# sholtodouglas/RoboticsPlayroomPybullet

Measured on AMD Instinct MI355X. Metric: env-steps/sec at N=4096 parallel UR5PlayAbsRPY1Obj-v0 envs per MI355X, higher is better.
Workload: dtype f32

## Files before the change

roboticsplayroompybullet_amd/csrc/rp_kernels.cuh:

```cuda
#pragma once
#include <hip/hip_runtime.h>
#include <stdint.h>

#include "rp_device_model.h"
#include "rp_math.cuh"

#define NB_MAX (1 + RP_MAX_ARM + RP_MAX_FREE + RP_MAX_J1)
#define NVP 28
#define MAXC 21
#define MAXACT 64
#define MAXT 4
#define MAXROWC (3 * MAXC + MAXT)
static_assert(MAXACT <= 64 && NB_MAX <= 32, "a candidate record packs its pair index in 6 bits and its bodies in 5 bits each");
#define PM_MAX 11
#define PMC_HDR 4
#define PMC_PT 11
#define PMC_MAN (8 + 4 * PMC_PT)
#define PMC_MANIFOLDS (PMC_HDR + PM_MAX * PMC_MAN)
#define PMC_AX PMC_MANIFOLDS
#define PMC_AXN 16
#define PMC_FLOATS (PMC_MANIFOLDS + 8 * PMC_AXN)
#define RP_MAX_GROUPS 16
#define SORT_KEYS 64
#define SORT_REPS 8
// ... 3 lines not shown
#define RP_MAX_ENVS (1 << SORT_RANK_BITS)
#define MAXSMALL 44

#ifndef RP_PREP_WAVES
#define RP_PREP_WAVES 4
#endif
#ifndef RP_WAVES_PER_EU
#define RP_WAVES_PER_EU 1
#endif

#define K_DT (1.0f / 300.0f)
#define K_GRAVITY (-9.8f)
#define K_NSUB 12
#define K_NSETTLE 100
#define K_MAXVEL 100.0f
#ifdef K_NITER_OVERRIDE
#define K_NITER K_NITER_OVERRIDE
#else
#define K_NITER 50
#endif
#define K_ERP 0.08f
#define K_SLOP 1e-5f
#define K_TIE_EPS 1e-6f
#define K_KP 0.1f
#define K_DEFMOTOR 1.0f
#define K_LIMIT_MAXIMP 100.0f
#define K_ERP_LIMIT 0.2f
#define K_LIMIT_ACTIVATION 0.1f
#define K_LIN_DAMP 0.04f
#define K_ANG_DAMP 0.04f
#define K_IK_DAMP 0.1f
#define K_IK_RES 1e-4f
#define K_IK_MAXSTEP (45.0f * RP_PI_F / 180.0f)

#define ROWW 18
#define ROWREG ((ROWW * MAXROWC + 3) & ~3)

#ifdef RP_WIDE
#define O_FLOATS 160
#else
#define O_FLOATS 128
#endif
#define CANDMAX 64
#define MANPTS (MAXC + 3)
#define NPSCR_FLOATS 768
#define PREP_CH 8

#define HULL_POOL_FIELDS int hinfo[MAXACT][4]; int hout[MAXACT]; float hpt[MAXACT][7]; unsigned long long hcls[PMC_AXN];
struct __align__(16) EnvLds {
  float st[RP_REC_FLOATS];
  float xR[NB_MAX * 9], xp[NB_MAX * 3];
  float O[4];
  float S[RP_MAX_ARM * 6];
  float Minv[144], tau[RP_MAX_ARM];
  float finv[RP_MAX_FREE * 9];
  float dmu[RP_MAX_OBJ], dmass[RP_MAX_FREE + 1];
  float vstar[32];
  float conp[MAXC * 3], conn[MAXC * 3], cond[MAXC], conmu[MAXC];
  int cona[MAXC], conb[MAXC], conk[MAXC];
  int torc[MAXT]; float tors[MAXT];
  alignas(16) float srow[MAXSMALL * 8];
  alignas(16) float rowS[MAXROWC * 4];
  alignas(16) float rowT[MAXROWC * 4];
  union alignas(16) {
    struct {
      float aabb[RP_MAX_COL * 8];
      int act[MAXACT], candn[MAXACT], key[MAXACT];
      float pmu[MAXACT];
      alignas(16) float cand[CANDMAX * 8];
      alignas(16) float man[MANPTS * 8];
      float npscr[NPSCR_FLOATS];
      HULL_POOL_FIELDS
    };
    struct {
      float inert[RP_MAX_ARM * 10], compI[RP_MAX_ARM * 10];
      float vsp[RP_MAX_ARM * 6], csp[RP_MAX_ARM * 6], fsp[RP_MAX_ARM * 6], Fv[RP_MAX_ARM * 6];
      double Md[144];
    };
    struct { float J[ROWREG]; float B[ROWREG]; };
  };
  alignas(16) float out[O_FLOATS];
};

struct __align__(16) PrepLds {
  float st[RP_REC_FLOATS];
  int roff[64];
  int slot[64];
  unsigned amask[4];
  int hdr[4];
  float O[4];
  float S[RP_MAX_ARM * 6];
  float xR[NB_MAX * 9], xp[NB_MAX * 3];
  float conp[MAXC * 3], conn[MAXC * 3], cond[MAXC], conmu[MAXC];
  int cona[MAXC], conb[MAXC], conk[MAXC];
  int torc[MAXT]; float tors[MAXT];
  union alignas(16) {
    float aabb[RP_MAX_COL * 8];
    float npscr[NPSCR_FLOATS];
    float man[MANPTS * 8];
  };
  int act[MAXACT], candn[MAXACT], key[MAXACT];
  float pmu[MAXACT];
  alignas(16) float cand[CANDMAX * 8];
  alignas(16) float Minv[144];
  float tau[RP_MAX_ARM];
  float finv[RP_MAX_FREE * 9];
  float dmu[RP_MAX_OBJ], dmass[RP_MAX_FREE + 1];
  float vstar[32];
  union alignas(16) {
    struct {
      float inert[RP_MAX_ARM * 10], compI[RP_MAX_ARM * 10];
      float vsp[RP_MAX_ARM * 6], csp[RP_MAX_ARM * 6], fsp[RP_MAX_ARM * 6], Fv[RP_MAX_ARM * 6];
      double Md[144];
    };
    struct {
      float srow[MAXSMALL * 8];
      float rowS[3 * PREP_CH * 4], rowT[3 * PREP_CH * 4];
      union {
        struct { float J[3 * PREP_CH * ROWW], B[3 * PREP_CH * ROWW]; };
        float aout[192];
      };
    };
  };
  HULL_POOL_FIELDS
#ifdef RP_LDS_PAD
  float pad[RP_LDS_PAD];
#endif
};
static_assert(offsetof(EnvLds, aabb) % 16 == 0 && offsetof(PrepLds, aabb) % 16 == 0 && offsetof(EnvLds, cand) % 16 == 0 && offsetof(EnvLds, man) % 16 == 0 && offsetof(EnvLds, srow) % 16 == 0 && offsetof(EnvLds, rowS) % 16 == 0 &&
              offsetof(EnvLds, rowT) % 16 == 0 && offsetof(EnvLds, J) % 16 == 0 && offsetof(EnvLds, B) % 16 == 0, "16-byte LDS accesses");
static_assert(sizeof(PrepLds) <= 20480 - 512, "k_prep2: eight blocks (sixteen waves: what its 128 VGPRs allow) per CU");
static_assert(offsetof(PrepLds, roff) % 16 == 0 && offsetof(PrepLds, slot) % 16 == 0 && offsetof(PrepLds, Minv) % 16 == 0 && offsetof(PrepLds, aout) % 16 == 0 &&
              offsetof(PrepLds, Md) % 8 == 0 && offsetof(PrepLds, cand) % 16 == 0 && offsetof(PrepLds, man) % 16 == 0, "16-byte copies out of LDS");

struct __align__(16) ObsLds {
  float st[RP_REC_FLOATS];
  float xR[NB_MAX * 9], xp[NB_MAX * 3];
  float O[4];
  float S[RP_MAX_ARM * 6];
  alignas(16) float cand[2 * 12 * RP_MAX_ARM + 2 * RP_MAX_ARM + 4];
  alignas(16) float out[O_FLOATS];
};
#ifdef RP_CLOCKS
__device__ unsigned long long g_clk[32 * 4096];
#define CLK_MARK(i) if (lane == 0) { g_clk[8 * wb + (i)] = __builtin_readcyclecounter(); }
#if RP_CLOCKS == 2
#define PCLK(i) if (lane == 0) { g_clk[32 * (blockIdx.x & 4095) + (i)] = (i) >= 6 && (i) < 8 ? wall_clock64() : __builtin_readcyclecounter(); }
#define PCLK_ZERO(i) if (lane == 0) { g_clk[32 * (blockIdx.x & 4095) + (i)] = 0ull; }
#define PCLK_ADD(i, v) if (lane == 0) { g_clk[32 * (blockIdx.x & 4095) + (i)] += (unsigned long long)(v); }
#define HCLK_ADD(i, v) if (l16 == 0) { atomicAdd(&g_clk[32 * (blockIdx.x & 4095) + (i)], (unsigned long long)(v)); }
#ifdef RP_HPROF
#define PCLK_G(i, v)
#define PCLK_H(i, v) PCLK_ADD(i, v)
#else
#define PCLK_G(i, v) PCLK_ADD(i, v)
#define PCLK_H(i, v)
#endif
#define CLK_MARK2(i)
#else
#define PCLK(i)
#define PCLK_ZERO(i)
#define PCLK_ADD(i, v)
#define HCLK_ADD(i, v)
#define PCLK_G(i, v)
#define PCLK_H(i, v)
#define CLK_MARK2(i) CLK_MARK(i)
#endif
#else
#define CLK_MARK(i)
#define CLK_MARK2(i)
#define PCLK(i)
#define PCLK_ZERO(i)
#define PCLK_ADD(i, v)
#define HCLK_ADD(i, v)
#define PCLK_G(i, v)
#define PCLK_H(i, v)
#endif

#define WSYNC() do { __builtin_amdgcn_fence(__ATOMIC_RELEASE, "workgroup"); __builtin_amdgcn_wave_barrier(); __builtin_amdgcn_fence(__ATOMIC_ACQUIRE, "workgroup"); } while (0)

__device__ __forceinline__ int dof_free(const DevModel* m, int k) { return m->n_arm + 6 * k; }
__device__ __forceinline__ int dof_j1(const DevModel* m, int k) { return m->n_arm + 6 * m->n_free + k; }
#ifndef RP_WIDE
#define LANE_J1 16
#define LANE_FREE 19
__device__ __forceinline__ int lane_pos(const DevModel* m, int d) {
  if (d < m->n_arm) return d;
  const int e = d - m->n_arm, f6 = 6 * m->n_free;
  if (e >= f6) return LANE_J1 + (e - f6);
  const int f = e / 6, c = e - 6 * f;
  if ((m->free_row0 >> f) & 1) return c < 3 ? m->n_arm + c : -1;
  return LANE_FREE + e;
}
__device__ __forceinline__ int lane_dof(const DevModel* m, int l) {
  if (l < 16) {
    if (l < m->n_arm) return l;
    const int c = l - m->n_arm;
    return (m->free_row0 != 0 && c < 3) ? m->n_arm + 6 * (__ffs(m->free_row0) - 1) + c : -1;
  }
  if (l >= 32) return -1;
  if (l < LANE_FREE) return l - LANE_J1 < m->n_j1 ? m->n_arm + 6 * m->n_free + (l - LANE_J1) : -1;
  const int e = l - LANE_FREE, f = e / 6;
  return (e < 6 * m->n_free && !((m->free_row0 >> f) & 1)) ? m->n_arm + e : -1;
}
#else
#define LANE_J1 16
#define LANE_FREE 19
__device__ __forceinline__ int lane_pos(const DevModel* m, int d) {
  if (d < m->n_arm) return d;
  const int e = d - m->n_arm, f6 = 6 * m->n_free;
  if (e >= f6) return LANE_J1 + (e - f6);
  const int f = e / 6, c = e - 6 * f;
  return f == m->drawer_free ? m->n_arm + c : LANE_FREE + 6 * f + c;
}
// ... 1790 lines not shown
        V3 rxn = tors ? d : cross(rr, d);
        float im = 1.f / L.dmass[k];
        M3 Ii = ldm3(&L.finv[9 * k]);
        V3 w = mulv(Ii, rxn);
        const V3 dl = tors ? mk3(0, 0, 0) : d;
        float jl[3] = {sign * dl.x, sign * dl.y, sign * dl.z}, ja[3] = {sign * rxn.x, sign * rxn.y, sign * rxn.z};
        float ba[3] = {sign * w.x, sign * w.y, sign * w.z};
        for (int i = 0; i < 3; i++) {
          J[base + i] = jl[i]; B[base + i] = jl[i] * im; J[base + 3 + i] = ja[i]; B[base + 3 + i] = ba[i];
          diag += jl[i] * jl[i] * im + ja[i] * ba[i];
          relv += jl[i] * L.vstar[dd + i] + ja[i] * L.vstar[dd + 3 + i];
        }
        if (base == 0) off0 = dd; else off1 = dd;
      } else {
        int k = body - 1 - n - m->n_free, dd = dof_j1(m, k);
        M3 R = ldm3(&L.xR[9 * body]);
        V3 a = mulv(R, ld3(m->j1_axis[k]));
        float j = tors ? (m->j1_type[k] == 1 ? 0.f : sign * dot(a, d)) : (m->j1_type[k] == 1 ? sign * dot(d, a) : sign * dot(a, cross(p - ld3(m->j1_pos[k]), d)));
        float minv = m->j1_minv[k];
        J[base] = j; B[base] = j * minv;
        diag += j * j * minv; relv += j * L.vstar[dd];
        if (base == 0) off0 = dd; else off1 = dd;
      }
    }
    if (has_arm) {
      off0 = 0;
#pragma unroll
      for (int k = 0; k < RP_MAX_ARM; k++) if (k < n) J[k] = Jr[k];
    }
    float* s = &L.rowS[4 * r];
    s[0] = diag; s[1] = relv; s[2] = dir == 0 ? 0.f : (tors ? L.tors[r - nc] : L.conmu[ci]); s[3] = __int_as_float(dir == 0 ? 0 : ci);
    float* t = &L.rowT[4 * r];
    t[0] = __int_as_float(has_arm ? 1 : 0); t[1] = dir == 0 ? 1e10f : 0.f; t[2] = __int_as_float(off0); t[3] = __int_as_float(off1);
  }
  WSYNC();
  for (int e = lane; e < nrows * n; e += 64) {
    int r = e / n, i = e - r * n;
    if (__float_as_int(L.rowT[4 * r]) != 0) {
      const float* J = &L.J[r * ROWW];
      const float* Mi = &L.Minv[i * 12];
      float b = 0.f;
#pragma unroll
      for (int k = 0; k < RP_MAX_ARM; k++) { const float t = Mi[k] * J[k]; b = k < n ? b + t : b; }
      L.B[r * ROWW + i] = b;
    }
  }
  WSYNC();
  for (int r = lane; r < nrows; r += 64) {
    float* s = &L.rowS[4 * r];
    float* t = &L.rowT[4 * r];
    float diag = s[0], relv = s[1];
    if (__float_as_int(t[0]) != 0) {
      const float* J = &L.J[r * ROWW];
      const float* B = &L.B[r * ROWW];
#pragma unroll
      for (int i = 0; i < RP_MAX_ARM; i++) { const float jb = J[i] * B[i], jv = J[i] * L.vstar[i]; diag = i < n ? diag + jb : diag; relv = i < n ? relv + jv : relv; }
    }
    float dinv, rhs, cfmr = 0.f;
    if (r < nc) {
      const int ci = c0 + r;
      float cfm = 0.f, erp = K_ERP;
      float s0 = m->col_stiff[L.cona[ci]], s1 = m->col_stiff[L.conb[ci]];
      if (s0 > 0.f || s1 > 0.f) {
        float d0 = s0 > 0.f ? m->col_damp[L.cona[ci]] : 0.1f, d1 = s1 > 0.f ? m->col_damp[L.conb[ci]] : 0.1f;
        if (!(s0 > 0.f)) s0 = 1e18f;
        if (!(s1 > 0.f)) s1 = 1e18f;
        float ks = 1.f / (1.f / s0 + 1.f / s1), kd = d0 + d1;
        cfm = 1.f / (K_DT * (K_DT * ks + kd));
        erp = (K_DT * ks) / (K_DT * ks + kd);
      }
      dinv = safe_inv(diag + cfm);
      cfmr = cfm * dinv;
      float pen = L.cond[ci] + K_SLOP, pos_err = 0.f, vel_err = -relv;
      if (pen > 0.f) vel_err -= pen / K_DT; else pos_err = -pen * erp / K_DT;
      rhs = (pos_err + vel_err) * dinv;
    } else { dinv = safe_inv(diag); rhs = -relv * dinv; }
    s[0] = rhs; s[1] = cfmr;
    t[0] = __int_as_float((__float_as_int(t[0]) != 0 && __float_as_int(t[3]) != 64) ? 1 : 0);
    float* Jw = &L.J[r * ROWW];
    for (int k = 0; k < ROWW; k++) Jw[k] *= dinv;
  }
}

__device__ __forceinline__ float pgs_update(float delta, float lam, float lo, float hi, float& lam_out) {
  float d = __builtin_amdgcn_fmed3f(delta, lo - lam, hi - lam);
  lam_out = lam + d;
  return d;
}

template <class LDS>
__device__ float solve_rows(const DevModel* m, LDS& L, int lane, int nsmall_, int ncon_, int nt_) {
  const int n = m->n_arm;
  const int nsmall = uni(nsmall_), nrc = uni(3 * ncon_ + nt_);
  float dv = 0.f;
  float lamS = 0.f, lamC0 = 0.f, lamC1 = 0.f;
  for (int it = 0; it < K_NITER; it++) {
    {
      for (int rr = 0; rr < nsmall; rr++) {
        const int r = (it & 1) ? rr : nsmall - 1 - rr;
        const float4 c0 = *(const float4*)&L.srow[8 * r], c1 = *(const float4*)&L.srow[8 * r + 4];
        const int type_ = uni(__float_as_int(c0.x)), dA = uni(__float_as_int(c0.y)), dB = uni(__float_as_int(c1.w));
        const int type = type_ == SR_LIMIT ? SR_UNIT : type_;
        const float sg = c0.z, jA = c1.x;
        float bl = 0.f;
        if (type == SR_J1) bl = lane == lane_pos(m, dA) ? sg : 0.f;
        else if (lane < n) bl = type == SR_UNIT ? sg * L.Minv[lane * 12 + dA] : L.Minv[lane * 12 + dA] + sg * L.Minv[lane * 12 + dB];
        float delta;
        if (type == SR_UNIT) delta = __fmaf_rn(-(sg * jA), lane_read(dv, dA), c0.w);
        else if (type == SR_J1) delta = __fmaf_rn(-jA, lane_read(dv, uni(lane_pos(m, dA))), c0.w);
        else { float pa = jA * lane_read(dv, dA); float pb = (sg * jA) * lane_read(dv, dB); float jdv = pa + pb; delta = c0.w - jdv; }
        float lam = lane_read(lamS, r), lnew;
        const float d = pgs_update(delta, lam, c1.y, c1.z, lnew);
        lamS = lane == r ? lnew : lamS;
        dv = fmaf(bl, d, dv);
      }
    }
    if (nrc > 0) {
      float4 sn = *(const float4*)&L.rowS[0], tn = *(const float4*)&L.rowT[0];
      float4 s2 = sn, t2 = tn;
      if (nrc > 1) { s2 = *(const float4*)&L.rowS[4]; t2 = *(const float4*)&L.rowT[4]; }
      float jn = 0.f, bn = 0.f;
      const int mydof = lane_dof(m, lane);
      {
        int i1 = mydof - __float_as_int(tn.w), i0 = mydof - __float_as_int(tn.z);
        int idx = (unsigned)i1 < 6u ? 12 + i1 : ((unsigned)i0 < 12u ? i0 : -1);
        if (idx >= 0 && mydof >= 0) { jn = L.J[idx]; bn = L.B[idx]; }
      }
      for (int r = 0; r < nrc; r++) {
        float jl = jn, bl = bn;
        float rhs = sn.x, cfmr = sn.y, mu = sn.z, lo_c = 0.f, hi_c = tn.y;
        int parent = uni(__float_as_int(sn.w));
        sn = s2; tn = t2;
        if (r + 1 < nrc) {
          int i1 = mydof - __float_as_int(tn.w), i0 = mydof - __float_as_int(tn.z);
          int idx = (unsigned)i1 < 6u ? 12 + i1 : ((unsigned)i0 < 12u ? i0 : -1);
          jn = 0.f; bn = 0.f;
          if (idx >= 0 && mydof >= 0) { jn = L.J[(r + 1) * ROWW + idx]; bn = L.B[(r + 1) * ROWW + idx]; }
          if (r + 2 < nrc) { s2 = *(const float4*)&L.rowS[4 * (r + 2)]; t2 = *(const float4*)&L.rowT[4 * (r + 2)]; }
        }
        float lamv = r < 64 ? lamC0 : lamC1;
        float lam = lane_read(lamv, r & 63);
        const float tot = lane_read(lamC0, parent);
        float lim = mu * tot;
        float prod = jl * dv;
        float jdv = wave_sum32(prod), lnew;
        float d = pgs_update(__fmaf_rn(-lam, cfmr, rhs) - jdv, lam, lo_c - lim, hi_c + lim, lnew);
        if (r >= uni(ncon_) && !(tot > 0.f)) { d = 0.f; lnew = lam; }
        float sel = lane == (r & 63) ? lnew : lamv;
        lamC0 = r < 64 ? sel : lamC0;
        lamC1 = r < 64 ? lamC1 : sel;
        dv = fmaf(bl, d, dv);
      }
    }
  }
  return dv;
}

__device__ bool substep_heavy(const DevModel* m, EnvLds& L, int lane, int nsmall, int ncon, int nt);
__device__ void substep(const DevModel* m, EnvLds& L, int lane, int env) {
  int n = m->n_arm;
  stage_dynamics(m, L, lane, env);
  fk_bodies(m, L, lane);
  __syncthreads();
  joint_subspaces(m, L, lane);
  collider_aabbs(m, L, lane);
  __syncthreads();
// ... 889 lines not shown
    float aj = 0.f;
#pragma unroll
    for (int j = 0; j < 7; j++) aj = l16 == j ? a8[j] : aj;
    qj = at == RP_ACT_REL_JOINTS ? aj + q0 : aj;
  } else {
    V3 cp = mk3(0, 0, 0); Q4 cq = {0.f, 0.f, 0.f, 1.f};
    if (at == RP_ACT_REL_RPY || at == RP_ACT_REL_QUAT) ee_pose_coop(m, qj, l16, cp, cq);
    V3 tpos; Q4 tq;
    action_target(at, a8, cp, cq, tpos, tq);
    if (m->arm_type == RP_ARM_PANDA) qj = ik_coop<7>(m, tpos, tq, qj, 200, l16, live, &ik_capped, &ik_marginal);
    else if (nc == 6) { for (int rep = 0; rep < 4; rep++) qj = ik_coop<6>(m, tpos, tq, qj, 20, l16, live, &ik_capped, &ik_marginal); }
    else { for (int rep = 0; rep < 4; rep++) qj = ik_coop<7>(m, tpos, tq, qj, 20, l16, live, &ik_capped, &ik_marginal); }
  }
  if (!live) return;
  if (l16 < nd) {
    float t = clampf(qj, m->ll[l16], m->ul[l16]);
    t = clampf(t, q0 - m->inc[l16], q0 + m->inc[l16]);
    st[ST_MMODE + l16] = 1.f; st[ST_MTARGET + l16] = t; st[ST_MMAXIMP + l16] = 240.f * K_DT;
    if (target_poses) target_poses[(size_t)env * nd + l16] = t;
  }
  if (l16 == 0) {
    st[ST_STATUS] = __int_as_float((ik_capped ? 8 : 0) | (ik_marginal ? 16 : 0));
    float g = a8[m->n_action - 1];
    if (m->arm_type == RP_ARM_PANDA) {
      float amt = 0.04f - g / 25.f;
      int ds[2] = {m->d9p, m->d10p};
      for (int i = 0; i < 2; i++) { st[ST_MMODE + ds[i]] = 1.f; st[ST_MTARGET + ds[i]] = amt; st[ST_MMAXIMP + ds[i]] = 100.f * K_DT; }
    } else {
      float amt = g - 0.2f;
      float left = st[ST_Q + m->d18];
      int ds[6] = {m->d18, m->d20, m->d12, m->d15, m->d10, m->d13};
      float tg[6] = {amt * 0.055f, left, amt * 0.5f, amt * 0.5f, amt * 0.8f, amt * 0.8f};
      float fo[6] = {100.f, 1000.f, 100.f, 100.f, 100.f, 100.f};
      for (int i = 0; i < 6; i++) { st[ST_MMODE + ds[i]] = 1.f; st[ST_MTARGET + ds[i]] = tg[i]; st[ST_MMAXIMP + ds[i]] = fo[i] * K_DT; }
    }
  }
}

__global__ void __launch_bounds__(64) k_action(const DevModel* __restrict__ m, float* __restrict__ state, const float* __restrict__ action,
                                              float* __restrict__ target_poses, int env0, int N, const int* __restrict__ member) {
  action_body(m, state, action, target_poses, env0, N, member, blockIdx.x);
}

__device__ __forceinline__ void copy_out(float* __restrict__ dst, const float* src, int nfloat, int lane) {
  for (int i = lane * 4; i < nfloat; i += 256) *(float4*)(dst + i) = *(const float4*)(src + i);
}

#define NBJ 3
#define LBL_N NBJ
#define NLBL (LBL_N + MAXC)
#define GEAR_LANE 12
#define W3_HDR 0
#define W3_VSTAR 8
#define W3_MU 40
#define W3_MINV 72
#define W3_A 216
#define W3_GEAR (W3_A + 160)
#define W3_ZERO (W3_GEAR + 7)
#define W3_BJ (W3_GEAR + 8)
#define W3_ROWS (W3_BJ + 20)
#define W3_ROWT (W3_ROWS + 4 * MAXROWC)
#define W3_ROFF (W3_ROWT + 4 * MAXROWC)
#define W3_SLOT (W3_ROFF + 64)
#define W3_J (W3_SLOT + 64)
#define W3_B (W3_J + ROWREG)
#define W3_SROW (W3_B + ROWREG)
#define W3_FLOATS (W3_SROW + 4 + 8 * MAXSMALL)
#define STAGE_FLOATS (128 + 2 * ROWREG)
#define AOUT_FLOATS (160 + 8 + 20)
static_assert(W3_A % 4 == 0 && W3_ROWS % 4 == 0 && W3_ROFF % 4 == 0 && AOUT_FLOATS % 4 == 0, "16-byte copies");

#define HV_MAXC 14
#ifndef S4_SLOTS0
#define S4_SLOTS0 8
#endif
#ifndef S4_SLOTS1
#define S4_SLOTS1 8
#endif
__device__ __forceinline__ int hv_class(int nc, int nA, int nB, int nC) {
  const bool heavy = nC != 0 || nA > S4_SLOTS0 || nB > S4_SLOTS1;
  return !heavy ? 0 : (nc <= HV_MAXC ? 1 : 2);
}
#define PREP_THREADS 128
__device__ __forceinline__ void prep2_core(PrepLds& L, const DevModel* __restrict__ m, const float* __restrict__ state, float* __restrict__ ws, const int env, const int cenv,
                                           int* __restrict__ pair_tab, const int pair_idx, int* __restrict__ hv_cnt = nullptr, int* __restrict__ hv_list = nullptr, const int prep_flags = 0) {
  const int tid = threadIdx.x, wid = tid >> 6, lane = tid & 63;
  PCLK(6) PCLK(0) PCLK_ZERO(15) PCLK_ZERO(19) PCLK_ZERO(26) PCLK_ZERO(27) PCLK_ZERO(28) PCLK_ZERO(29) PCLK_ZERO(30) PCLK_ZERO(31)
  static_assert(RP_REC_FLOATS == PREP_THREADS, "one float of the record per thread");
  L.st[tid] = state[(size_t)env * RP_REC_FLOATS + tid];
  if (tid == 64) L.hdr[3] = pair_idx;
  if (tid == 64 && m->persist) L.hdr[2] = __float_as_int(m->pmcache[(size_t)cenv * PMC_FLOATS]);
  stage_dynamics(m, L, tid, cenv);
  __syncthreads();
  PCLK(16)
  if (wid == 0) fk_bodies(m, L, lane);
  __syncthreads();
  PCLK(17)
  float* w = ws + (size_t)env * W3_FLOATS;
  if (wid == 0) {
    collider_aabbs(m, L, lane);
    WSYNC();
    PCLK(1)
    int ncon = collide<PrepLds>(m, L, lane, cenv, &L.hdr[2]);
    ncon = uni(ncon);
#ifdef RP_ABL_MAXCON
    if (ncon > RP_ABL_MAXCON) ncon = RP_ABL_MAXCON;
#endif
    if (lane == 0) L.hdr[0] = ncon;
    PCLK(2)
  } else {
    joint_subspaces(m, L, lane);
    PCLK(18)
    arm_dynamics(m, L, lane, cenv);
    unconstrained_velocities(m, L, lane, cenv);
    PCLK(3)
    int nsmall = build_small_rows(m, L, lane);
    nsmall = uni(nsmall);
    for (int i = lane; i < AOUT_FLOATS; i += 64) L.aout[i] = 0.f;
    if (lane < 2) L.amask[lane] = 0u;
    if (lane == 2) L.amask[2] = (unsigned)nsmall;
    WSYNC();
    bool gear = false;
    if (lane < nsmall) {
      const float* s = &L.srow[8 * lane];
      int type = __float_as_int(s[0]), dA = __float_as_int(s[1]);
      float sg = s[2], rhs = s[3], dinv = s[4], lo = s[5], hi = s[6];
      if (type == SR_UNIT) {
        L.aout[dA] = dinv; L.aout[16 + dA] = rhs; L.aout[32 + dA] = lo; L.aout[48 + dA] = hi;
      } else if (type == SR_LIMIT) {
        int pl = sg > 0.f ? 64 : 112;
        L.aout[pl + dA] = sg * rhs; L.aout[pl + 16 + dA] = sg * lo; L.aout[pl + 32 + dA] = sg * hi;
        atomicOr(&L.amask[sg > 0.f ? 0 : 1], 1u << dA);
      } else if (type == SR_J1) {
        int k = lane;
        if (k < NBJ) { float* bq = &L.aout[168]; bq[k] = dinv; bq[4 + k] = rhs; bq[8 + k] = lo; bq[12 + k] = hi; bq[16 + k] = sg; }
      } else {
        float* g = &L.aout[160];
        g[0] = s[1]; g[1] = s[7]; g[2] = sg; g[3] = dinv; g[4] = rhs; g[5] = lo; g[6] = hi;
        gear = true;
      }
    }
    const bool anygear = __ballot(gear) != 0ull;
    if (lane == 0) L.hdr[1] = anygear ? 1 : 0;
    WSYNC();
    if (lane < 32) w[W3_VSTAR + lane] = L.vstar[lane];
    copy_out(w + W3_MINV, L.Minv, 144, lane);
    copy_out(w + W3_A, L.aout, AOUT_FLOATS, lane);
  }
  __syncthreads();
  const int ncon = L.hdr[0];
  int tid_j = threadIdx.x;
  asm volatile("" : "+v"(tid_j));
  const int wid_j = tid_j >> 6;
  if (wid_j == 0) {
    const int lane = tid_j & 63;
    float* w = ws + (size_t)env * W3_FLOATS;
    const int cls = lane < ncon ? L.conk[lane] : 3;
    const unsigned long long mB = __ballot(cls == 0), mA = __ballot(cls == 1), mC = __ballot(cls == 2);
    const unsigned long long lower = (1ull << lane) - 1ull;
    L.slot[lane] = -1;
    L.roff[lane] = 0;
    const int nt = tors_list(m, L, lane, ncon);
    WSYNC();
    if (cls == 0) L.slot[__popcll(mB & lower)] = lane;
    else if (cls == 1) L.slot[21 + __popcll(mA & lower)] = lane;
    else if (cls == 2) L.slot[42 + __popcll(mC & lower)] = lane;
    bool tors_done = nt == 0;
    for (int c0 = 0; c0 < ncon || !tors_done; c0 += PREP_CH) {
      const int nc = max(0, min(PREP_CH, ncon - c0));
      const int ntl = (!tors_done && c0 + PREP_CH >= ncon && 3 * nc + nt <= 3 * PREP_CH) ? nt : 0;
      contact_rows(m, L, lane, c0, nc, ntl);
      WSYNC();
      auto global_row = [&](int lr) { return lr < nc ? c0 + lr : (lr < nc + ntl ? 3 * ncon + (lr - nc) : ncon + 2 * c0 + (lr - nc - ntl)); };
      for (int e = lane; e < (3 * nc + ntl) * ROWW; e += 64) {
        const int lr = e / ROWW, k = e - lr * ROWW;
        const int gr = global_row(lr);
        w[W3_J + gr * ROWW + k] = L.J[e]; w[W3_B + gr * ROWW + k] = L.B[e];
      }
      for (int e = lane; e < (3 * nc + ntl) * 4; e += 64) {
        const int lr = e >> 2, k = e & 3;
        const int gr = global_row(lr);
        float v = L.rowS[e];
        if (k == 3 && lr >= nc && lr < nc + ntl) {
          const int c = L.torc[lr - nc], kc = L.conk[c];
          const unsigned long long mk = kc == 1 ? mA : (kc == 2 ? mC : mB);
          v = __int_as_float(c | (kc << 8) | (__popcll(mk & ((1ull << c) - 1ull)) << 12));
        }
        w[W3_ROWS + gr * 4 + k] = v; w[W3_ROWT + gr * 4 + k] = L.rowT[e];
      }
      if (lane < 3 * nc + ntl && !(lane >= nc && lane < nc + ntl)) {
        const int gr = global_row(lane);
        L.roff[gr] = __float_as_int(L.rowT[4 * lane + 2]) | (__float_as_int(L.rowT[4 * lane + 3]) << 8);
      }
      if (ntl > 0) tors_done = true;
      WSYNC();
    }
    PCLK(4)
    if (lane == 0) {
      int nj = m->n_j1 < NBJ ? m->n_j1 : NBJ;
      w[W3_HDR] = __int_as_float((int)L.amask[0]); w[W3_HDR + 1] = __int_as_float((int)L.amask[1]);
      w[W3_HDR + 2] = __int_as_float(nj); w[W3_HDR + 3] = __int_as_float(ncon);
      w[W3_HDR + 4] = __int_as_float(__popcll(mA)); w[W3_HDR + 5] = __int_as_float(__popcll(mB));
      w[W3_HDR + 6] = __int_as_float(L.hdr[1] | (nt << 8)); w[W3_HDR + 7] = __int_as_float(__popcll(mC));
      if (hv_list != nullptr && (hv_class(ncon, __popcll(mA), __popcll(mB), __popcll(mC)) != 0 || (prep_flags & 1))) hv_list[atomicAdd(hv_cnt, 1)] = env | (ncon << 24);
    }
    if (lane < 32) w[W3_MU + lane] = lane < ncon ? L.conmu[lane] : 0.f;
    copy_out(w + W3_ROFF, (const float*)L.roff, 64, lane);
    copy_out(w + W3_SLOT, (const float*)L.slot, 64, lane);
  } else {
    if ((tid_j & 63) == 0) pair_tab[L.hdr[3]] = env | (ncon << 24);
    if (prep_flags & 1) {
      const int lane = tid_j & 63;
      float* w = ws + (size_t)env * W3_FLOATS;
      const int nsm = (int)L.amask[2];
      if (lane == 0) w[W3_SROW] = __int_as_float(nsm);
      for (int i = lane; i < 8 * nsm; i += 64) w[W3_SROW + 4 + i] = L.srow[i];
    }
  }
  PCLK(5) PCLK(7)
}
__device__ __forceinline__ void prep2_body(const DevModel* __restrict__ m, const float* __restrict__ state, float* __restrict__ ws, int env0, int N,
                                           const int* __restrict__ sort_cnt, int* __restrict__ sort_cnt_next, const int* __restrict__ sort_slot, int* __restrict__ pair_env,
                                           const int* __restrict__ member, const int bid, const int* __restrict__ cache_env = nullptr, int* __restrict__ hv_cnt = nullptr, int* __restrict__ hv_cnt_next = nullptr,
                                           int* __restrict__ hv_list = nullptr, const int prep_flags = 0) {
  __shared__ PrepLds L;
  const int tid = threadIdx.x, wid = tid >> 6, lane = tid & 63;
  int env = env0 + bid;
  if (env >= N) return;
  if (member) env = member[env];
  if (bid == 0) {
    for (int i = tid; i < SORT_BINS; i += PREP_THREADS) sort_cnt_next[i] = 0;
    if (tid == 0 && hv_cnt_next) *hv_cnt_next = 0;
  }
  int pair_place = 0;
  if (wid == 1) {
    const int my_slot = sort_slot[env];
    int cnt8[8];
#pragma unroll
    for (int t = 0; t < 8; t++) cnt8[t] = sort_cnt[8 * lane + t];
    const int mybin = my_slot >> SORT_RANK_BITS;
    int above = 0;
#pragma unroll
    for (int t = 0; t < 8; t++) above += (8 * lane + t > mybin) ? cnt8[t] : 0;
#pragma unroll
    for (int d = 32; d >= 1; d >>= 1) above += __shfl_xor(above, d);
    pair_place = above + (my_slot & SORT_RANK_MASK);
  }
  prep2_core(L, m, state, ws, env, cache_env ? cache_env[env] : env, pair_env, env0 + pair_place, hv_cnt, hv_list ? hv_list + env0 : nullptr, prep_flags);
}
#define PREP2_ARGS const DevModel* __restrict__ m, const float* __restrict__ state, float* __restrict__ ws, int env0, int N, \
                   const int* __restrict__ sort_cnt, int* __restrict__ sort_cnt_next, const int* __restrict__ sort_slot, int* __restrict__ pair_env, \
                   const int* __restrict__ member
#define HV_ARGS int* __restrict__ hv_cnt, int* __restrict__ hv_cnt_next, int* __restrict__ hv_list, int prep_flags
__global__ void __launch_bounds__(PREP_THREADS, RP_PREP_WAVES) k_prep2(PREP2_ARGS, HV_ARGS) { prep2_body(m, state, ws, env0, N, sort_cnt, sort_cnt_next, sort_slot, pair_env, member, blockIdx.x, nullptr, hv_cnt, hv_cnt_next, hv_list, prep_flags); }
__global__ void __launch_bounds__(PREP_THREADS, RP_PREP_WAVES) k_settle_prep(PREP2_ARGS, const int* __restrict__ cache_env, int prep_flags) { prep2_body(m, state, ws, env0, N, sort_cnt, sort_cnt_next, sort_slot, pair_env, member, blockIdx.x, cache_env, nullptr, nullptr, nullptr, prep_flags); }
__global__ void __launch_bounds__(PREP_THREADS, RP_PREP_WAVES) k_action_prep(const DevModel* __restrict__ m, float* __restrict__ state, float* __restrict__ ws, int env0, int N,
                                                                   const int* __restrict__ sort_cnt, int* __restrict__ sort_cnt_next, const int* __restrict__ sort_slot,
                                                                   int* __restrict__ pair_env, const int* __restrict__ member, const float* __restrict__ action,
                                                                   float* __restrict__ target_poses, int nab, HV_ARGS) {
  if ((int)blockIdx.x < nab) {
    __builtin_amdgcn_s_setprio(3);
    action_body(m, state, action, target_poses, env0, N, member, blockIdx.x);
  }
  else prep2_body(m, state, ws, env0, N, sort_cnt, sort_cnt_next, sort_slot, pair_env, member, blockIdx.x - nab, nullptr, hv_cnt, hv_cnt_next, hv_list, prep_flags);
}


typedef float f16v __attribute__((ext_vector_type(16)));
__device__ __forceinline__ float row16_sum(float v) {
  int x = __float_as_int(v);
  v += __int_as_float(__builtin_amdgcn_update_dpp(0, x, 0xB1, 0xF, 0xF, true));
  x = __float_as_int(v);
  v += __int_as_float(__builtin_amdgcn_update_dpp(0, x, 0x4E, 0xF, 0xF, true));
  x = __float_as_int(v);
  v += __int_as_float(__builtin_amdgcn_update_dpp(0, x, 0x141, 0xF, 0xF, true));
  x = __float_as_int(v);
  v += __int_as_float(__builtin_amdgcn_update_dpp(0, x, 0x140, 0xF, 0xF, true));
  return v;
}
__device__ __forceinline__ float fold_rows(float v) {
  unsigned u = __float_as_uint(v);
  auto sw = __builtin_amdgcn_permlane16_swap(u, u, false, false);
  return __uint_as_float(sw[0]) + __uint_as_float(sw[1]);
}
struct Plane { float rhs, lo, hi, lam, dacc, loP, hiP; };
struct PlaneN : Plane { float cfm, rhsE; };
#define PLANE_FENCE4(a, b, c, d) asm volatile("s_nop 1" : "+v"((a).loP), "+v"((a).hiP), "+v"((b).loP), "+v"((b).hiP), "+v"((c).loP), "+v"((c).hiP), "+v"((d).loP), "+v"((d).hiP))
#define PLANE_FENCE_N(a, b, c) asm volatile("s_nop 1" : "+v"((a).loP), "+v"((a).hiP), "+v"((b).rhsE), "+v"((c).rhsE))
__device__ __forceinline__ void plane_begin(Plane& p) { p.loP = p.lo - p.lam; p.hiP = p.hi - p.lam; p.dacc = 0.f; }
__device__ __forceinline__ void plane_end(Plane& p) { p.lam += p.dacc; }
__device__ __forceinline__ void nplane_begin(PlaneN& p) { p.loP = p.lo - p.lam; p.hiP = p.hi - p.lam; p.dacc = 0.f; p.rhsE = __fmaf_rn(-p.lam, p.cfm, p.rhs); }
__device__ __forceinline__ void fplane_begin(Plane& p, float lim, float tot) {
  const bool on = tot > 0.f;
  p.loP = on ? (0.f - lim) - p.lam : 0.f; p.hiP = on ? (0.f + lim) - p.lam : 0.f; p.dacc = 0.f;
}

#define DPP_ALL " row_mask:0xf bank_mask:0xf bound_ctrl:1\n"

template <int I>
// ... 1467 lines not shown
```

Before: 2.131 million.

## Split contact-row preparation across both prep waves with double-buffered LDS chunks

The contact-row build in k_prep2 used to run on wave 0 alone while wave 1 sat idle. Now each wave builds one of two chunks at a time, and the second chunk buffer sits in the collision scratch, which is dead after the join. The waves then split the global writes: one stores J and rowS, the other B and rowT, using 8- and 16-byte vector stores instead of scalar stores. This adds block-wide barriers per chunk pair, a zero-fill of the first chunk, and a more intricate LDS union layout that risks aliasing mistakes.

```diff
diff --git a/roboticsplayroompybullet_amd/csrc/rp_kernels.cuh b/roboticsplayroompybullet_amd/csrc/rp_kernels.cuh
--- a/roboticsplayroompybullet_amd/csrc/rp_kernels.cuh
+++ b/roboticsplayroompybullet_amd/csrc/rp_kernels.cuh
@@ -109,6 +109,10 @@
   alignas(16) float out[O_FLOATS];
 };
 
+struct __align__(16) PrepChunk {
+  float rowS[3 * PREP_CH * 4], rowT[3 * PREP_CH * 4];
+  float J[3 * PREP_CH * ROWW], B[3 * PREP_CH * ROWW];
+};
 struct __align__(16) PrepLds {
   float st[RP_REC_FLOATS];
   int roff[64];
@@ -122,13 +126,18 @@
   int cona[MAXC], conb[MAXC], conk[MAXC];
   int torc[MAXT]; float tors[MAXT];
   union alignas(16) {
-    float aabb[RP_MAX_COL * 8];
-    float npscr[NPSCR_FLOATS];
-    float man[MANPTS * 8];
+    struct {
+      union alignas(16) {
+        float aabb[RP_MAX_COL * 8];
+        float npscr[NPSCR_FLOATS];
+        float man[MANPTS * 8];
+      };
+      int act[MAXACT], candn[MAXACT], key[MAXACT];
+      float pmu[MAXACT];
+      alignas(16) float cand[CANDMAX * 8];
+    };
+    PrepChunk ch1;
   };
-  int act[MAXACT], candn[MAXACT], key[MAXACT];
-  float pmu[MAXACT];
-  alignas(16) float cand[CANDMAX * 8];
   alignas(16) float Minv[144];
   float tau[RP_MAX_ARM];
   float finv[RP_MAX_FREE * 9];
@@ -142,10 +151,9 @@
     };
     struct {
       float srow[MAXSMALL * 8];
-      float rowS[3 * PREP_CH * 4], rowT[3 * PREP_CH * 4];
       union {
-        struct { float J[3 * PREP_CH * ROWW], B[3 * PREP_CH * ROWW]; };
-        float aout[192];
+        PrepChunk ch0;
+        struct { float rows_[2 * 3 * PREP_CH * 4]; float aout[192]; };
       };
     };
   };
@@ -157,6 +165,11 @@
 static_assert(offsetof(EnvLds, aabb) % 16 == 0 && offsetof(PrepLds, aabb) % 16 == 0 && offsetof(EnvLds, cand) % 16 == 0 && offsetof(EnvLds, man) % 16 == 0 && offsetof(EnvLds, srow) % 16 == 0 && offsetof(EnvLds, rowS) % 16 == 0 &&
               offsetof(EnvLds, rowT) % 16 == 0 && offsetof(EnvLds, J) % 16 == 0 && offsetof(EnvLds, B) % 16 == 0, "16-byte LDS accesses");
 static_assert(sizeof(PrepLds) <= 20480 - 512, "k_prep2: eight blocks (sixteen waves: what its 128 VGPRs allow) per CU");
+static_assert(offsetof(PrepLds, ch1) == offsetof(PrepLds, aabb) && offsetof(PrepLds, ch1) + sizeof(PrepChunk) <= offsetof(PrepLds, cand) + sizeof(PrepLds::cand) &&
+              offsetof(PrepLds, cand) + sizeof(PrepLds::cand) <= offsetof(PrepLds, Minv), "the second chunk of contact rows lies inside the collision wave's scratch, dead after the join");
+static_assert(offsetof(PrepLds, ch0) % 16 == 0 && offsetof(PrepLds, ch1) % 16 == 0 && offsetof(PrepChunk, rowT) % 16 == 0 && offsetof(PrepChunk, J) % 16 == 0 && offsetof(PrepChunk, B) % 16 == 0 &&
+              (3 * PREP_CH * ROWW) % 4 == 0 && ROWW % 2 == 0 && offsetof(PrepLds, aout) == offsetof(PrepLds, ch0) + offsetof(PrepChunk, J) && sizeof(PrepLds::aout) <= sizeof(PrepChunk::J),
+              "16-byte zero-fill and row copies, 8-byte copies of the compact rows; aout lies over the first chunk's J");
 static_assert(offsetof(PrepLds, roff) % 16 == 0 && offsetof(PrepLds, slot) % 16 == 0 && offsetof(PrepLds, Minv) % 16 == 0 && offsetof(PrepLds, aout) % 16 == 0 &&
               offsetof(PrepLds, Md) % 8 == 0 && offsetof(PrepLds, cand) % 16 == 0 && offsetof(PrepLds, man) % 16 == 0, "16-byte copies out of LDS");
 
@@ -2113,6 +2126,152 @@
   }
 }
 
+__device__ __forceinline__ void prep_rows(const DevModel* m, PrepLds& L, PrepChunk& C, int lane, int c0, int nc, int nt, bool zero) {
+  const int n = m->n_arm;
+  const int nrows = 3 * nc + nt;
+  V3 O = ld3(L.O);
+  if (zero) {
+    for (int i = 4 * lane; i < nrows * ROWW; i += 256) { *(float4*)&C.J[i] = make_float4(0.f, 0.f, 0.f, 0.f); *(float4*)&C.B[i] = make_float4(0.f, 0.f, 0.f, 0.f); }
+    WSYNC();
+  }
+  for (int r = lane; r < nrows; r += 64) {
+    int ci, dir;
+    if (r < nc) { ci = c0 + r; dir = 0; }
+    else if (r < nc + nt) { ci = L.torc[r - nc]; dir = 3; }
+    else { ci = c0 + ((r - nc - nt) >> 1); dir = 1 + ((r - nc - nt) & 1); }
+    V3 nrm = ld3(&L.conn[3 * ci]);
+    const V3 pmid = ld3(&L.conp[3 * ci]);
+    const V3 half = nrm * (0.5f * L.cond[ci]);
+    V3 d = nrm;
+    const bool tors = dir == 3;
+    if (dir == 1 || dir == 2) {
+      V3 t1, t2;
+      if (fabsf(nrm.z) > 0.7071067811865475244f) {
+        float a = nrm.y * nrm.y + nrm.z * nrm.z, k = 1.f / sqrtf(a);
+        t1 = mk3(0.f, -nrm.z * k, nrm.y * k);
+        t2 = mk3(a * k, -nrm.x * t1.z, nrm.x * t1.y);
+      } else {
+        float a = nrm.x * nrm.x + nrm.y * nrm.y, k = 1.f / sqrtf(a);
+        t1 = mk3(-nrm.y * k, nrm.x * k, 0.f);
+        t2 = mk3(-nrm.z * t1.y, nrm.z * t1.x, a * k);
+      }
+      d = dir == 1 ? t1 : t2;
+    }
+    float* J = &C.J[r * ROWW];
+    float* B = &C.B[r * ROWW];
+    bool has_arm = false;
+    float diag = 0.f, relv = 0.f;
+    int off0 = 64, off1 = 64;
+    int bodyA = m->col_body[L.cona[ci]], bodyB = m->col_body[L.conb[ci]];
+    bool any_arm = (bodyA >= 1 && bodyA <= n) || (bodyB >= 1 && bodyB <= n);
+    int nother = 0;
+    float Jr[RP_MAX_ARM];
+#pragma unroll
+    for (int k = 0; k < RP_MAX_ARM; k++) Jr[k] = 0.f;
+    for (int side = 0; side < 2; side++) {
+      int body = side == 0 ? bodyA : bodyB;
+      float sign = side == 0 ? 1.f : -1.f;
+      if (body == 0) continue;
+      const V3 p = side == 0 ? pmid + half : pmid - half;
+      if (body <= n) {
+        V6 f; f.a = tors ? d : cross(p - O, d); f.l = tors ? mk3(0, 0, 0) : d;
+        uint32_t anc = m->arm_anc[body - 1];
+#pragma unroll
+        for (int k = 0; k < RP_MAX_ARM; k++) {
+          const float v = sign * dot6(ld6(&L.S[6 * k]), f);
+          Jr[k] = (k < n && ((anc >> k) & 1u)) ? Jr[k] + v : Jr[k];
+        }
+        has_arm = true;
+        continue;
+      }
+      int base = (any_arm || nother == 1) ? 12 : 0;
+      nother++;
+      if (body <= n + m->n_free) {
+        int k = body - 1 - n, dd = dof_free(m, k);
+        V3 rr = p - ld3(&L.st[ST_FREE + 13 * k]);
+        V3 rxn = tors ? d : cross(rr, d);
+        float im = 1.f / L.dmass[k];
+        M3 Ii = ldm3(&L.finv[9 * k]);
+        V3 w = mulv(Ii, rxn);
+        const V3 dl = tors ? mk3(0, 0, 0) : d;
+        float jl[3] = {sign * dl.x, sign * dl.y, sign * dl.z}, ja[3] = {sign * rxn.x, sign * rxn.y, sign * rxn.z};
+        float ba[3] = {sign * w.x, sign * w.y, sign * w.z};
+        for (int i = 0; i < 3; i++) {
+          J[base + i] = jl[i]; B[base + i] = jl[i] * im; J[base + 3 + i] = ja[i]; B[base + 3 + i] = ba[i];
+          diag += jl[i] * jl[i] * im + ja[i] * ba[i];
+          relv += jl[i] * L.vstar[dd + i] + ja[i] * L.vstar[dd + 3 + i];
+        }
+        if (base == 0) off0 = dd; else off1 = dd;
+      } else {
+        int k = body - 1 - n - m->n_free, dd = dof_j1(m, k);
+        M3 R = ldm3(&L.xR[9 * body]);
+        V3 a = mulv(R, ld3(m->j1_axis[k]));
+        float j = tors ? (m->j1_type[k] == 1 ? 0.f : sign * dot(a, d)) : (m->j1_type[k] == 1 ? sign * dot(d, a) : sign * dot(a, cross(p - ld3(m->j1_pos[k]), d)));
+        float minv = m->j1_minv[k];
+        J[base] = j; B[base] = j * minv;
+        diag += j * j * minv; relv += j * L.vstar[dd];
+        if (base == 0) off0 = dd; else off1 = dd;
+      }
+    }
+    if (has_arm) {
+      off0 = 0;
+#pragma unroll
+      for (int k = 0; k < RP_MAX_ARM; k++) if (k < n) J[k] = Jr[k];
+    }
+    float* s = &C.rowS[4 * r];
+    s[0] = diag; s[1] = relv; s[2] = dir == 0 ? 0.f : (tors ? L.tors[r - nc] : L.conmu[ci]); s[3] = __int_as_float(dir == 0 ? 0 : ci);
+    float* t = &C.rowT[4 * r];
+    t[0] = __int_as_float(has_arm ? 1 : 0); t[1] = dir == 0 ? 1e10f : 0.f; t[2] = __int_as_float(off0); t[3] = __int_as_float(off1);
+  }
+  WSYNC();
+  for (int e = lane; e < nrows * n; e += 64) {
+    int r = e / n, i = e - r * n;
+    if (__float_as_int(C.rowT[4 * r]) != 0) {
+      const float* J = &C.J[r * ROWW];
+      const float* Mi = &L.Minv[i * 12];
+      float b = 0.f;
+#pragma unroll
+      for (int k = 0; k < RP_MAX_ARM; k++) { const float t = Mi[k] * J[k]; b = k < n ? b + t : b; }
+      C.B[r * ROWW + i] = b;
+    }
+  }
+  WSYNC();
+  for (int r = lane; r < nrows; r += 64) {
+    float* s = &C.rowS[4 * r];
+    float* t = &C.rowT[4 * r];
+    float diag = s[0], relv = s[1];
+    if (__float_as_int(t[0]) != 0) {
+      const float* J = &C.J[r * ROWW];
+      const float* B = &C.B[r * ROWW];
+#pragma unroll
+      for (int i = 0; i < RP_MAX_ARM; i++) { const float jb = J[i] * B[i], jv = J[i] * L.vstar[i]; diag = i < n ? diag + jb : diag; relv = i < n ? relv + jv : relv; }
+    }
+    float dinv, rhs, cfmr = 0.f;
+    if (r < nc) {
+      const int ci = c0 + r;
+      float cfm = 0.f, erp = K_ERP;
+      float s0 = m->col_stiff[L.cona[ci]], s1 = m->col_stiff[L.conb[ci]];
+      if (s0 > 0.f || s1 > 0.f) {
+        float d0 = s0 > 0.f ? m->col_damp[L.cona[ci]] : 0.1f, d1 = s1 > 0.f ? m->col_damp[L.conb[ci]] : 0.1f;
+        if (!(s0 > 0.f)) s0 = 1e18f;
+        if (!(s1 > 0.f)) s1 = 1e18f;
+        float ks = 1.f / (1.f / s0 + 1.f / s1), kd = d0 + d1;
+        cfm = 1.f / (K_DT * (K_DT * ks + kd));
+        erp = (K_DT * ks) / (K_DT * ks + kd);
+      }
+      dinv = safe_inv(diag + cfm);
+      cfmr = cfm * dinv;
+      float pen = L.cond[ci] + K_SLOP, pos_err = 0.f, vel_err = -relv;
+      if (pen > 0.f) vel_err -= pen / K_DT; else pos_err = -pen * erp / K_DT;
+      rhs = (pos_err + vel_err) * dinv;
+    } else { dinv = safe_inv(diag); rhs = -relv * dinv; }
+    s[0] = rhs; s[1] = cfmr;
+    t[0] = __int_as_float((__float_as_int(t[0]) != 0 && __float_as_int(t[3]) != 64) ? 1 : 0);
+    float* Jw = &C.J[r * ROWW];
+    for (int k = 0; k < ROWW; k++) Jw[k] *= dinv;
+  }
+}
+
 __device__ __forceinline__ float pgs_update(float delta, float lam, float lo, float hi, float& lam_out) {
   float d = __builtin_amdgcn_fmed3f(delta, lo - lam, hi - lam);
   lam_out = lam + d;
@@ -3168,6 +3327,8 @@
   return !heavy ? 0 : (nc <= HV_MAXC ? 1 : 2);
 }
 #define PREP_THREADS 128
+static_assert((W3_J * 4) % 16 == 0 && (W3_B * 4) % 16 == 0 && (W3_ROWS * 4) % 16 == 0 && (W3_ROWT * 4) % 16 == 0 && (W3_FLOATS * 4) % 16 == 0 && (ROWW * 4) % 8 == 0,
+              "k_prep2 stores the compact rows 8 bytes and rowS / rowT 16 bytes at a time");
 __device__ __forceinline__ void prep2_core(PrepLds& L, const DevModel* __restrict__ m, const float* __restrict__ state, float* __restrict__ ws, const int env, const int cenv,
                                            int* __restrict__ pair_tab, const int pair_idx, int* __restrict__ hv_cnt = nullptr, int* __restrict__ hv_list = nullptr, const int prep_flags = 0) {
   const int tid = threadIdx.x, wid = tid >> 6, lane = tid & 63;
@@ -3232,75 +3393,103 @@
     if (lane < 32) w[W3_VSTAR + lane] = L.vstar[lane];
     copy_out(w + W3_MINV, L.Minv, 144, lane);
     copy_out(w + W3_A, L.aout, AOUT_FLOATS, lane);
+    WSYNC();
+    for (int i = 4 * lane; i < 3 * PREP_CH * ROWW; i += 256) { *(float4*)&L.ch0.J[i] = make_float4(0.f, 0.f, 0.f, 0.f); *(float4*)&L.ch0.B[i] = make_float4(0.f, 0.f, 0.f, 0.f); }
   }
   __syncthreads();
-  const int ncon = L.hdr[0];
+  const int ncon = uni(L.hdr[0]);
   int tid_j = threadIdx.x;
   asm volatile("" : "+v"(tid_j));
-  const int wid_j = tid_j >> 6;
-  if (wid_j == 0) {
+  const int wid_j = uni(tid_j >> 6);
+  {
     const int lane = tid_j & 63;
+    if (wid_j == 0) { PCLK(12) }
     float* w = ws + (size_t)env * W3_FLOATS;
     const int cls = lane < ncon ? L.conk[lane] : 3;
     const unsigned long long mB = __ballot(cls == 0), mA = __ballot(cls == 1), mC = __ballot(cls == 2);
-    const unsigned long long lower = (1ull << lane) - 1ull;
-    L.slot[lane] = -1;
-    L.roff[lane] = 0;
-    const int nt = tors_list(m, L, lane, ncon);
-    WSYNC();
-    if (cls == 0) L.slot[__popcll(mB & lower)] = lane;
-    else if (cls == 1) L.slot[21 + __popcll(mA & lower)] = lane;
-    else if (cls == 2) L.slot[42 + __popcll(mC & lower)] = lane;
-    bool tors_done = nt == 0;
-    for (int c0 = 0; c0 < ncon || !tors_done; c0 += PREP_CH) {
-      const int nc = max(0, min(PREP_CH, ncon - c0));
-      const int ntl = (!tors_done && c0 + PREP_CH >= ncon && 3 * nc + nt <= 3 * PREP_CH) ? nt : 0;
-      contact_rows(m, L, lane, c0, nc, ntl);
+    if (wid_j == 0) {
+      const unsigned long long lower = (1ull << lane) - 1ull;
+      L.slot[lane] = -1;
+      L.roff[lane] = 0;
+      const int ntw = tors_list(m, L, lane, ncon);
+      if (lane == 0) L.amask[3] = (unsigned)ntw;
       WSYNC();
-      auto global_row = [&](int lr) { return lr < nc ? c0 + lr : (lr < nc + ntl ? 3 * ncon + (lr - nc) : ncon + 2 * c0 + (lr - nc - ntl)); };
-      for (int e = lane; e < (3 * nc + ntl) * ROWW; e += 64) {
-        const int lr = e / ROWW, k = e - lr * ROWW;
-        const int gr = global_row(lr);
-        w[W3_J + gr * ROWW + k] = L.J[e]; w[W3_B + gr * ROWW + k] = L.B[e];
-      }
-      for (int e = lane; e < (3 * nc + ntl) * 4; e += 64) {
-        const int lr = e >> 2, k = e & 3;
-        const int gr = global_row(lr);
-        float v = L.rowS[e];
-        if (k == 3 && lr >= nc && lr < nc + ntl) {
-          const int c = L.torc[lr - nc], kc = L.conk[c];
-          const unsigned long long mk = kc == 1 ? mA : (kc == 2 ? mC : mB);
-          v = __int_as_float(c | (kc << 8) | (__popcll(mk & ((1ull << c) - 1ull)) << 12));
+      if (cls == 0) L.slot[__popcll(mB & lower)] = lane;
+      else if (cls == 1) L.slot[21 + __popcll(mA & lower)] = lane;
+      else if (cls == 2) L.slot[42 + __popcll(mC & lower)] = lane;
+    }
+    __syncthreads();
+    const int nt = uni((int)L.amask[3]);
+    const int jl = ncon > 0 ? (ncon - 1) / PREP_CH : 0, jt = nt == 0 ? -1 : (3 * (ncon - PREP_CH * jl) + nt <= 3 * PREP_CH ? jl : jl + 1);
+    const int nchunk = max(jt + 1, (ncon + PREP_CH - 1) / PREP_CH);
+    for (int j0 = 0; j0 < nchunk; j0 += 2) {
+      if (j0 > 0) __syncthreads();
+      const int c0a = PREP_CH * j0, c0b = c0a + PREP_CH;
+      const int nca = max(0, min(PREP_CH, ncon - c0a)), ncb = max(0, min(PREP_CH, ncon - c0b));
+      const int nta = j0 == jt ? nt : 0, ntb = j0 + 1 == jt ? nt : 0;
+      {
+        const int c0 = wid_j ? c0b : c0a, nc = wid_j ? ncb : nca, ntl = wid_j ? ntb : nta;
+        if (3 * nc + ntl > 0) {
+          PrepChunk& C = wid_j ? L.ch1 : L.ch0;
+          const float* cT = C.rowT;
+          prep_rows(m, L, C, lane, c0, nc, ntl, wid_j != 0 || j0 > 0);
+          WSYNC();
+          if (lane < 3 * nc + ntl && !(lane >= nc && lane < nc + ntl)) {
+            const int gr = lane < nc ? c0 + lane : ncon + 2 * c0 + (lane - nc - ntl);
+            L.roff[gr] = __float_as_int(cT[4 * lane + 2]) | (__float_as_int(cT[4 * lane + 3]) << 8);
+          }
         }
-        w[W3_ROWS + gr * 4 + k] = v; w[W3_ROWT + gr * 4 + k] = L.rowT[e];
-      }
-      if (lane < 3 * nc + ntl && !(lane >= nc && lane < nc + ntl)) {
-        const int gr = global_row(lane);
-        L.roff[gr] = __float_as_int(L.rowT[4 * lane + 2]) | (__float_as_int(L.rowT[4 * lane + 3]) << 8);
-      }
-      if (ntl > 0) tors_done = true;
-      WSYNC();
-    }
-    PCLK(4)
-    if (lane == 0) {
-      int nj = m->n_j1 < NBJ ? m->n_j1 : NBJ;
-      w[W3_HDR] = __int_as_float((int)L.amask[0]); w[W3_HDR + 1] = __int_as_float((int)L.amask[1]);
-      w[W3_HDR + 2] = __int_as_float(nj); w[W3_HDR + 3] = __int_as_float(ncon);
-      w[W3_HDR + 4] = __int_as_float(__popcll(mA)); w[W3_HDR + 5] = __int_as_float(__popcll(mB));
-      w[W3_HDR + 6] = __int_as_float(L.hdr[1] | (nt << 8)); w[W3_HDR + 7] = __int_as_float(__popcll(mC));
-      if (hv_list != nullptr && (hv_class(ncon, __popcll(mA), __popcll(mB), __popcll(mC)) != 0 || (prep_flags & 1))) hv_list[atomicAdd(hv_cnt, 1)] = env | (ncon << 24);
-    }
-    if (lane < 32) w[W3_MU + lane] = lane < ncon ? L.conmu[lane] : 0.f;
-    copy_out(w + W3_ROFF, (const float*)L.roff, 64, lane);
-    copy_out(w + W3_SLOT, (const float*)L.slot, 64, lane);
-  } else {
-    if ((tid_j & 63) == 0) pair_tab[L.hdr[3]] = env | (ncon << 24);
-    if (prep_flags & 1) {
-      const int lane = tid_j & 63;
-      float* w = ws + (size_t)env * W3_FLOATS;
-      const int nsm = (int)L.amask[2];
-      if (lane == 0) w[W3_SROW] = __int_as_float(nsm);
-      for (int i = lane; i < 8 * nsm; i += 64) w[W3_SROW + 4 + i] = L.srow[i];
+      }
+      __syncthreads();
+      if (wid_j == 0) { PCLK(20) }
+      {
+        float2* dst = (float2*)(w + (wid_j ? W3_B : W3_J));
+        for (int h = 0; h < 2; h++) {
+          const PrepChunk& C = h ? L.ch1 : L.ch0;
+          const float2* src = (const float2*)(wid_j ? C.B : C.J);
+          const int c0 = h ? c0b : c0a, nc = h ? ncb : nca, ntl = h ? ntb : nta;
+          const int e1 = nc * (ROWW / 2), e2 = (nc + ntl) * (ROWW / 2), e3 = (3 * nc + ntl) * (ROWW / 2);
+          const int g1 = c0 * (ROWW / 2), g2 = (3 * ncon - nc) * (ROWW / 2), g3 = (ncon + 2 * c0 - nc - ntl) * (ROWW / 2);
+          for (int e = lane; e < e3; e += 64) dst[e + (e < e1 ? g1 : (e < e2 ? g2 : g3))] = src[e];
+        }
+      }
+      {
+        const int h = lane >> 5, lr = lane & 31;
+        const int c0 = h ? c0b : c0a, nc = h ? ncb : nca, ntl = h ? ntb : nta;
+        if (lr < 3 * nc + ntl) {
+          const int gr = lr < nc ? c0 + lr : (lr < nc + ntl ? 3 * ncon + (lr - nc) : ncon + 2 * c0 + (lr - nc - ntl));
+          const PrepChunk& C = h ? L.ch1 : L.ch0;
+          const float* src = wid_j ? C.rowT : C.rowS;
+          float4 v = *(const float4*)&src[4 * lr];
+          if (wid_j == 0 && lr >= nc && lr < nc + ntl) {
+            const int c = L.torc[lr - nc], kc = L.conk[c];
+            const unsigned long long mk = kc == 1 ? mA : (kc == 2 ? mC : mB);
+            v.w = __int_as_float(c | (kc << 8) | (__popcll(mk & ((1ull << c) - 1ull)) << 12));
+          }
+          *(float4*)&w[(wid_j ? W3_ROWT : W3_ROWS) + 4 * gr] = v;
+        }
+      }
+    }
+    if (wid_j == 0) {
+      PCLK(4)
+      if (lane == 0) {
+        int nj = m->n_j1 < NBJ ? m->n_j1 : NBJ;
+        w[W3_HDR] = __int_as_float((int)L.amask[0]); w[W3_HDR + 1] = __int_as_float((int)L.amask[1]);
+        w[W3_HDR + 2] = __int_as_float(nj); w[W3_HDR + 3] = __int_as_float(ncon);
+        w[W3_HDR + 4] = __int_as_float(__popcll(mA)); w[W3_HDR + 5] = __int_as_float(__popcll(mB));
+        w[W3_HDR + 6] = __int_as_float(L.hdr[1] | (nt << 8)); w[W3_HDR + 7] = __int_as_float(__popcll(mC));
+        if (hv_list != nullptr && (hv_class(ncon, __popcll(mA), __popcll(mB), __popcll(mC)) != 0 || (prep_flags & 1))) hv_list[atomicAdd(hv_cnt, 1)] = env | (ncon << 24);
+      }
+      if (lane < 32) w[W3_MU + lane] = lane < ncon ? L.conmu[lane] : 0.f;
+      copy_out(w + W3_ROFF, (const float*)L.roff, 64, lane);
+      copy_out(w + W3_SLOT, (const float*)L.slot, 64, lane);
+    } else {
+      if (lane == 0) pair_tab[L.hdr[3]] = env | (ncon << 24);
+      if (prep_flags & 1) {
+        const int nsm = (int)L.amask[2];
+        if (lane == 0) w[W3_SROW] = __int_as_float(nsm);
+        for (int i = lane; i < 8 * nsm; i += 64) w[W3_SROW + 4 + i] = L.srow[i];
+      }
     }
   }
   PCLK(5) PCLK(7)
```

Result: slower. 2.094 million (-1.8%).
